# sunzeyucmu/VAE-based-Music--Deep-Generative-Models

Hardware: AMD Instinct MI355X
Metric: audio-samples/sec/GPU VQ-VAE train step, 44.1kHz 65536-frame chunks @1/2/4/8 GPU (higher is better)
Workload: dtype bf16; 1 GPU; SMALL_VQ_VAE 3-level VQ-VAE train step (BASELINE config 2); model=VQVAE levels=3 latent=64 K=2048 down_depth=[3,2,2] width=32 depth=4 dil=3, global_batch=32, seq_len=65536, parallelism=dp1, graph=True

## Files before the change

include/vqa.h:

```cpp
#ifndef VQA_H
#define VQA_H

#include <stddef.h>
#include <stdint.h>

#ifdef __cplusplus
extern "C" {
#endif

typedef void* vqa_stream_t;

enum { VQA_OK = 0, VQA_E_INVALID_ARG = -1, VQA_E_UNSUPPORTED = -2, VQA_E_HIP = -3 };
enum { VQA_F32 = 0, VQA_BF16 = 1 };

enum {
  VQA_PRE_RELU = 1,
  VQA_ADD_RESIDUAL = 2,
  VQA_POST_MASK = 4,
  VQA_X_F32 = 8,
  VQA_Y_F32 = 16
};

const char* vqa_get_last_error(void);
const char* vqa_version(void);
// ... 34 lines not shown
  float* db;
  int nparts;
  int n;
  int n_w;
  int reserved;
} vqa_partials_desc;
int vqa_conv1d_bwd_weight_partials(const void* x, const void* dy, float* dw, float* db, int B, int T_in, int T_out,
                                   int C_in, int C_out, int K, int stride, int dilation, int pad_left, int flags,
                                   int dtype, void* workspace, size_t ws_bytes, vqa_partials_desc* desc,
                                   vqa_stream_t stream);
int vqa_conv1d_transpose_bwd_weight_partials(const void* x, const void* dy, float* dw, float* db, int B, int T_in,
                                             int T_out, int C_in, int C_out, int K, int stride, int pad_left,
                                             int flags, int dtype, void* workspace, size_t ws_bytes,
                                             vqa_partials_desc* desc, vqa_stream_t stream);
int vqa_reduce_partials(const vqa_partials_desc* descs, int count, vqa_stream_t stream);

int vqa_conv1d_bwd_data_weight(const void* dy, const float* w, const void* x, const void* residual, void* dx,
                               float* dw, float* db, int B, int T_in, int T_out, int C_in, int C_out, int K,
                               int stride, int dilation, int pad_left, int flags, int dtype, void* workspace,
                               size_t ws_bytes, vqa_partials_desc* desc, vqa_stream_t stream);
size_t vqa_conv1d_bwd_data_weight_workspace(int B, int T_in, int T_out, int C_in, int C_out, int K, int stride,
                                            int dilation, int pad_left, int flags, int dtype);

enum {
  VQA_OP_FWD = 0, VQA_OP_BWD_DATA = 1, VQA_OP_BWD_WEIGHT = 2, VQA_OP_BWD_DATA_WEIGHT = 3,
  VQA_OP_T_FWD = 4, VQA_OP_T_BWD_DATA = 5, VQA_OP_T_BWD_WEIGHT = 6
};
enum {
  VQA_ROUTE_CO1 = 0, VQA_ROUTE_CONV32 = 1, VQA_ROUTE_GATHER_MFMA = 2, VQA_ROUTE_CI1 = 3, VQA_ROUTE_THIN_O = 4,
  VQA_ROUTE_THIN = 5, VQA_ROUTE_DIRECT = 6, VQA_ROUTE_WGRAD_MFMA = 7, VQA_ROUTE_WGRAD_THIN = 8,
// ... 259 lines not shown
```

vae-based-music--deep-generative-models_amd/csrc/vqa_conv.h:

```cpp
#pragma once
#include "vqa_common.h"

namespace vqa {

enum { W_DIRECT = 0, W_FLIP_T = 1, W_PAIR = 2 };

struct GatherArgs {
  const void* x;
  const float* w;
  const float* bias;
  const void* resid;
  const void* mask;
  void* y;
  int B, T_in, T_out;
  int C, O;
  int K, S, D, P;
  int wmode, Kb, Pb;
  int T_full;
  int flags;
  float* wpart = nullptr;
  int wrelu = 0;
  int wbf16 = 0;
};

// ... 58 lines not shown

enum { G_CONV32, G_MFMA, G_CI1, G_THINO, G_THIN, G_DIRECT };
struct GatherRoute {
  int family;
  int pvx;
  MfmaPlan m;
};

enum { WG_MFMA = 0, WG_THIN_X = 1, WG_THIN_G = 2, WG_DIRECT = 3 };
struct WgradPlan {
  int kind;
  int TT, CH, nchunk, nwg, E, nb;
  size_t lds, ws_bytes;
};

int gather_check(const GatherArgs& a, int dtype);
GatherRoute gather_route(const GatherArgs& a, int dtype);
int gather_nep(const GatherArgs& a, bool fw);
bool gather_thin_fits(const GatherArgs& a);
int conv32_pvx(const GatherArgs& a, int dtype, bool fw);
int run_gather(const GatherArgs& a, int dtype, hipStream_t s);
int launch_conv32_fused(const GatherArgs& a, int pvx, int dtype, hipStream_t s, int* nwg);

int wgrad_route(WgradPlan* out, int dtype, int B, int T_in, int T_out, int C, int O, int K, int S, int D, int flags);
int run_wgrad(const void* x, const void* g, float* dw, float* db, int B, int T_in, int T_out, int C, int O, int K,
              int S, int D, int P, int flags, int dtype, void* ws, size_t ws_bytes, hipStream_t s,
              vqa_partials_desc* defer);
size_t wgrad_ws(int dtype, int B, int T_in, int T_out, int C, int O, int K, int S, int D, int flags);
int reduce_partials(const float* ws, int nparts, int E, int n_w, float* dw, float* db, hipStream_t s);

}
```

vae-based-music--deep-generative-models_amd/csrc/vqa_conv.hip:

```cpp
#include "vqa_conv.h"
#include "vqa_launch.h"
#include <algorithm>

using namespace vqa;

extern "C" int vqa_same_out_len(int T_in, int stride) {
  if (stride < 1 || T_in < 0) return -1;
  return (T_in + stride - 1) / stride;
}
extern "C" int vqa_same_pad_left(int T_in, int K, int stride, int dilation) {
  if (stride < 1 || dilation < 1 || K < 1 || T_in < 0) return -1;
  const int out = (T_in + stride - 1) / stride;
  const int pad = std::max((out - 1) * stride + (K - 1) * dilation + 1 - T_in, 0);
  return pad / 2;
}

static GatherArgs conv_fwd_gather(const void* x, const float* w, const float* bias, const void* residual, void* y,
                                  int B, int T_in, int T_out, int C_in, int C_out, int K, int stride, int dilation,
                                  int pad_left, int flags) {
  return GatherArgs{x, w, bias, residual, nullptr, y, B, T_in, T_out, C_in, C_out, K, stride, dilation, pad_left,
                    W_DIRECT, K, 0, T_out, flags & (VQA_PRE_RELU | VQA_ADD_RESIDUAL | VQA_X_F32 | VQA_Y_F32)};
}

static int swap_xy_flags(int flags) {
// ... 146 lines not shown
                   conv_wgrad_flags(flags), dtype, workspace, ws_bytes, (hipStream_t)stream,
                   desc);
}

extern "C" int vqa_conv1d_transpose_bwd_weight_partials(const void* x, const void* dy, float* dw, float* db, int B,
                                                        int T_in, int T_out, int C_in, int C_out, int K, int stride,
                                                        int pad_left, int flags, int dtype, void* workspace,
                                                        size_t ws_bytes, vqa_partials_desc* desc,
                                                        vqa_stream_t stream) {
  VQA_ARG(desc, "bwd_weight_partials: NULL descriptor");
  if (const int rc = convT_check(K, stride, pad_left)) return rc;
  VQA_ARG(T_out == stride * T_in, "conv1d_transpose_bwd_weight: T_out %d != stride*T_in", T_out);
  const int f = convT_wgrad_flags(flags);
  return run_wgrad(dy, x, dw, db, B, T_out, T_in, C_out, C_in, K, stride, 1, pad_left, f, dtype, workspace, ws_bytes,
                   (hipStream_t)stream, desc);
}

static size_t fused_bwd_ws(int C_in, int C_out, int K) {
  return (size_t)cu_count() * kMaxGatherPerCU * (size_t)(K * C_in * C_out + C_out) * sizeof(float);
}

static GatherArgs fused_bwd_args(const void* dy, const float* w, const void* x, const void* residual, void* dx, int B,
                                 int T_in, int T_out, int C_in, int C_out, int K, int dilation, int pad_left,
                                 int flags) {
  const bool relu = flags & VQA_PRE_RELU;
  const int f = swap_xy_flags(flags & (VQA_ADD_RESIDUAL | VQA_X_F32 | VQA_Y_F32)) | (relu ? VQA_POST_MASK : 0);
  GatherArgs a{dy, w, nullptr, residual, x, dx, B, T_out, T_in, C_out, C_in, K, 1, dilation,
               (K - 1) * dilation - pad_left, W_FLIP_T, K, 0, T_in, f};
  a.wrelu = relu ? 1 : 0;
  return a;
// ... 205 lines not shown
```

vae-based-music--deep-generative-models_amd/csrc/vqa_conv_wgrad.hip:

```cpp
#include "vqa_conv.h"
#include "vqa_launch.h"
#include "vqa_mfma.h"

namespace vqa {

template <class T, int C, int PV>
struct RowStager {
  static constexpr int VEC = 16 / (int)sizeof(T), CPR = C / VEC;
  uint4 v[PV];
  unsigned ok;
  __device__ __forceinline__ void load(const T* Xi, int lo, int hi, int r0, int rows) {
    ok = 0u;
#pragma unroll
    for (int i = 0; i < PV; ++i) {
      const int e = threadIdx.x + i * 256;
      const int rr = e / CPR, q = e - rr * CPR, ti = r0 + rr;
      const bool val = e < rows * CPR && ti >= lo && ti < hi;
      const int tc = val ? ti : lo;
      v[i] = *((const uint4*)(Xi + (long long)tc * C) + (val ? q : 0));
      ok |= val ? (1u << i) : 0u;
    }
  }
  __device__ __forceinline__ void store(T* xl, int XS, int rows, bool relu) {
#pragma unroll
// ... 8 lines not shown
      }
    }
  }
  __device__ __forceinline__ void tail(T* xl, int XS, const T* Xi, int lo, int hi, int r0, int rows, bool relu) {
    for (int e = threadIdx.x + PV * 256; e < rows * CPR; e += 256) {
      const int rr = e / CPR, q = e - rr * CPR, ti = r0 + rr;
      uint4 t = {0u, 0u, 0u, 0u};
      if (ti >= lo && ti < hi) t = *((const uint4*)(Xi + (long long)ti * C) + q);
      if (relu) relu_bits<T>(t);
      *(uint4*)(xl + rr * XS + q * VEC) = t;
    }
  }
};

template <class T, int C, int O, int TT>
__global__ __launch_bounds__(256) void wgrad_mfma_kernel(WgradArgs a) {
  typedef Mfma<T> M;
  constexpr int XS = C + lds_pad<T>();
  constexpr int GS = O + lds_pad<T>();
  constexpr int CT = C / 16, OT = O / 16;
  constexpr int MAXTW = CT * OT;
  constexpr int KT = (int)sizeof(T) == 2 ? 32 : 4;
  extern __shared__ __attribute__((aligned(16))) char smem[];
  T* gl = (T*)smem;
  T* xl = gl + TT * GS;
  __shared__ float red[256];

  const int n = blockIdx.y, ch = blockIdx.x;
  const int tbeg = ch * a.CH, tend = min(a.T_out, tbeg + a.CH);
  const int rows_in = (TT - 1) * a.S + (a.K - 1) * a.D + 1;
  const int ntile = a.K * CT * OT;
  const int wave = __builtin_amdgcn_readfirstlane(threadIdx.x >> 6), lane = threadIdx.x & 63;

  f32x4 acc[MAXTW];
#pragma unroll
  for (int i = 0; i < MAXTW; ++i) acc[i] = f32x4{0.f, 0.f, 0.f, 0.f};
  float dbacc = 0.f;
  const bool db_x = a.flags & WG_DB_FROM_X;
  const int NB = db_x ? C : O;
  const int dbo = threadIdx.x % NB, dbr = threadIdx.x / NB, dbstep = 256 / NB;

  const bool relu = a.flags & VQA_PRE_RELU;
  const T* Gi = (const T*)a.g + (long long)n * a.T_out * O;
// ... 62 lines not shown
      for (int r = 0; r < 4; ++r) {
        const int c = ct * 16 + 4 * (lane >> 4) + r;
        out[((size_t)k * C + c) * O + o] = acc[ti][r];
      }
    }
  }
  red[threadIdx.x] = dbacc;
  __syncthreads();
  if (threadIdx.x < NB) {
    float s = 0.f;
    for (int r = 0; r < dbstep; ++r) s += red[r * NB + threadIdx.x];
    out[a.K * C * O + threadIdx.x] = s;
  }
}


template <class T> __device__ __forceinline__ float ld1_buf(__amdgpu_buffer_rsrc_t r, int off);
template <> __device__ __forceinline__ float ld1_buf<float>(__amdgpu_buffer_rsrc_t r, int off) {
  return __builtin_bit_cast(float, __builtin_amdgcn_raw_buffer_load_b32(r, off, 0, 0));
}
template <> __device__ __forceinline__ float ld1_buf<bf16>(__amdgpu_buffer_rsrc_t r, int off) {
  return __uint_as_float((unsigned)__builtin_amdgcn_raw_buffer_load_b16(r, off, 0, 0) << 16);
}
template <class T> __device__ __forceinline__ void ld8_buf(__amdgpu_buffer_rsrc_t r, int off, float* v);
template <> __device__ __forceinline__ void ld8_buf<bf16>(__amdgpu_buffer_rsrc_t r, int off, float* v) {
  const u32x4 w = __builtin_amdgcn_raw_buffer_load_b128(r, off, 0, 0);
#pragma unroll
  for (int i = 0; i < 4; ++i) {
    v[2 * i] = __uint_as_float(w[i] << 16);
    v[2 * i + 1] = __uint_as_float(w[i] & 0xFFFF0000u);
  }
}
template <> __device__ __forceinline__ void ld8_buf<float>(__amdgpu_buffer_rsrc_t r, int off, float* v) {
  const u32x4 a = __builtin_amdgcn_raw_buffer_load_b128(r, off, 0, 0);
  const u32x4 b = __builtin_amdgcn_raw_buffer_load_b128(r, off + 16, 0, 0);
#pragma unroll
  for (int i = 0; i < 4; ++i) {
    v[i] = __uint_as_float(a[i]);
    v[i + 4] = __uint_as_float(b[i]);
  }
}

template <class TX, class TG, bool WIDE_X, int NM>
__global__ __launch_bounds__(256) void wgrad_thin_kernel(WgradArgs a) {
  constexpr int KM = 4, U = 8;
  const int W = WIDE_X ? a.C : a.O;
  const int NN = WIDE_X ? a.O : a.C;
  const int VL = W / 8, RL = 256 / VL;
  const int v = threadIdx.x % VL, rl = threadIdx.x / VL;
  const int n = blockIdx.y, ch = blockIdx.x;
  const int tbeg = ch * a.CH, tend = min(a.T_out, tbeg + a.CH);
  const bool relu = a.flags & VQA_PRE_RELU;
  const unsigned xbytes = (unsigned)a.T_in * a.C * (unsigned)sizeof(TX), gbytes = (unsigned)a.T_out * a.O * (unsigned)sizeof(TG);
  const __amdgpu_buffer_rsrc_t rx = item_rsrc(a.x, (long long)n * xbytes, xbytes);
  const __amdgpu_buffer_rsrc_t rg = item_rsrc(a.g, (long long)n * gbytes, gbytes);
  float acc[KM][NM][8];
  float bacc[8];
#pragma unroll
  for (int k = 0; k < KM; ++k)
#pragma unroll
    for (int i = 0; i < NM; ++i)
#pragma unroll
      for (int j = 0; j < 8; ++j) acc[k][i][j] = 0.f;
#pragma unroll
  for (int j = 0; j < 8; ++j) bacc[j] = 0.f;
// ... 78 lines not shown
      const int o = e % a.O, c = (e / a.O) % a.C, k = e / (a.O * a.C);
      const int wide = WIDE_X ? c : o, narrow = WIDE_X ? o : c;
      vv = wide / 8;
      q = (k * NM + narrow) * 8 + (wide % 8);
    } else {
      const int o = e - KCO;
      vv = WIDE_X ? 0 : o / 8;
      q = KM * NM * 8 + (WIDE_X ? o : o % 8);
    }
    float sum = 0.f;
    for (int r = 0; r < RL; ++r) sum += red[(r * VL + vv) * PER + q];
    out[e] = sum;
  }
}

template <class TX, class TG, int TT>
__global__ __launch_bounds__(256) void wgrad_direct_kernel(WgradArgs a) {
  extern __shared__ __attribute__((aligned(16))) char smem[];
  float* gl = (float*)smem;
  float* xl = gl + TT * a.O;
  constexpr int EPT = 16;
  const int n = blockIdx.y, ch = blockIdx.x;
  const int tbeg = ch * a.CH, tend = min(a.T_out, tbeg + a.CH);
  const int rows_in = (TT - 1) * a.S + (a.K - 1) * a.D + 1;
  const int E = a.K * a.C * a.O;
  const int e0 = blockIdx.z * EPT * 256;
  const bool relu = a.flags & VQA_PRE_RELU;
  float acc[EPT];
#pragma unroll
  for (int i = 0; i < EPT; ++i) acc[i] = 0.f;
  float dbacc = 0.f;
  for (int t0 = tbeg; t0 < tend; t0 += TT) {
    const int nrows = min(TT, tend - t0);
    for (int e = threadIdx.x; e < TT * a.O; e += blockDim.x) {
      const int r = e / a.O, o = e - r * a.O;
      gl[e] = r < nrows ? ld((const TG*)a.g + ((long long)n * a.T_out + t0 + r) * a.O + o) : 0.f;
    }
    for (int e = threadIdx.x; e < rows_in * a.C; e += blockDim.x) {
      const int r = e / a.C, c = e - r * a.C;
      const int ti = t0 * a.S - a.P + r;
      float v = (ti >= 0 && ti < a.T_in) ? ld((const TX*)a.x + ((long long)n * a.T_in + ti) * a.C + c) : 0.f;
      xl[e] = relu ? fmaxf(v, 0.f) : v;
    }
    __syncthreads();
    if (blockIdx.z == 0) {
      if (a.flags & WG_DB_FROM_X) {
        if (threadIdx.x < a.C)
          for (int r = a.P; r < a.P + nrows * a.S; ++r) dbacc += xl[r * a.C + threadIdx.x];
      } else if (threadIdx.x < a.O) {
        for (int r = 0; r < nrows; ++r) dbacc += gl[r * a.O + threadIdx.x];
      }
    }
#pragma unroll
    for (int i = 0; i < EPT; ++i) {
      const int e = e0 + threadIdx.x + i * 256;
      if (e < E) {
        const int o = e % a.O, c = (e / a.O) % a.C, k = e / (a.O * a.C);
        float s = acc[i];
        for (int r = 0; r < nrows; ++r) s += xl[(r * a.S + k * a.D) * a.C + c] * gl[r * a.O + o];
        acc[i] = s;
      }
    }
    __syncthreads();
  }
  float* out = a.ws + (size_t)(n * a.nchunk + ch) * (size_t)(E + a.nb);
#pragma unroll
  for (int i = 0; i < EPT; ++i) {
    const int e = e0 + threadIdx.x + i * 256;
    if (e < E) out[e] = acc[i];
  }
  if (blockIdx.z == 0 && threadIdx.x < a.nb) out[E + threadIdx.x] = dbacc;
}

constexpr int kRedCols = 16;
__device__ __forceinline__ float reduce_col16(const float* ws, int nparts, int E, int e, float (*red)[kRedCols]) {
  const int el = threadIdx.x & (kRedCols - 1), grp = threadIdx.x / kRedCols;
  float s[8] = {0.f, 0.f, 0.f, 0.f, 0.f, 0.f, 0.f, 0.f};
  if (e < E) {
    int p = grp;
    for (; p + 7 * 16 < nparts; p += 8 * 16)
#pragma unroll
      for (int u = 0; u < 8; ++u) s[u] += ws[(size_t)(p + 16 * u) * E + e];
    for (; p < nparts; p += 16) s[0] += ws[(size_t)p * E + e];
  }
  red[grp][el] = ((s[0] + s[1]) + (s[2] + s[3])) + ((s[4] + s[5]) + (s[6] + s[7]));
  __syncthreads();
// ... 236 lines not shown
      typedef tag_t<decltype(tg)> TG;
      if (p.kind == WG_THIN_X) return launch_wgrad_thin<TX, TG, true>(a, p, s);
      if (p.kind == WG_THIN_G) return launch_wgrad_thin<TX, TG, false>(a, p, s);
      return launch_wgrad_direct<TX, TG>(a, p, s);
    });
  }
  if (rc != VQA_OK) return rc;
  const int KCO = K * C * O;
  if (defer) {
    *defer = vqa_partials_desc{(const float*)ws, dw, db, p.nwg, p.E, KCO, 0};
    return VQA_OK;
  }
  return reduce_partials((const float*)ws, p.nwg, p.E, KCO, dw, db, s);
}

size_t wgrad_ws(int dtype, int B, int T_in, int T_out, int C, int O, int K, int S, int D, int flags) {
  if (B < 1 || T_in < 1 || T_out < 1 || C < 1 || O < 1 || K < 1 || S < 1 || D < 1) return 0;
  return plan_wgrad(dtype, B, T_in, T_out, C, O, K, S, D, flags).ws_bytes;
}

}

using namespace vqa;

extern "C" int vqa_reduce_partials(const vqa_partials_desc* descs, int count, vqa_stream_t stream) {
  VQA_ARG(count >= 0 && (count == 0 || descs), "reduce_partials: bad descriptor list");
  for (int base = 0; base < count; base += kMaxDescs) {
    ReduceBatch rb{};
    rb.count = count - base < kMaxDescs ? count - base : kMaxDescs;
    int blocks = 0;
// ... 19 lines not shown
```

vae-based-music--deep-generative-models_amd/vqa_layers.py:

```python
from __future__ import annotations

import math
from typing import Dict, List, Optional, Tuple

import numpy as np
import torch

import vqa_lib as V


class ParamStore:

    ALIGN = 4

    def __init__(self):
        self.specs: List[Tuple[str, Tuple[int, ...], str]] = []
        self.offsets: Dict[str, Tuple[int, Tuple[int, ...]]] = {}
        self.size = 0
        self.count = 0
        self.flat: Optional[torch.Tensor] = None
        self.grad: Optional[torch.Tensor] = None
        self.deferred = None

    def add(self, name: str, shape: Tuple[int, ...], init: str) -> str:
# ... 158 lines not shown
    def backward_data(self, dy, T_in, cdt, mask=None, residual=None, out_dtype=None):
        B, To, _ = dy.shape
        xdt = out_dtype or cdt
        dx = torch.empty((B, T_in, self.cin), dtype=xdt, device=dy.device)
        fl = _flags_for(dx, dy.dtype, cdt) | (V.POST_MASK if mask is not None else 0) | \
            (V.ADD_RESIDUAL if residual is not None else 0)
        V.conv1d_bwd_data(dy, self.w, mask, residual, dx, B, T_in, To, self.cin, self.cout, self.K, self.s, self.d,
                          self.pad(T_in), fl, V.dtype_code(cdt))
        return dx

    def backward_weight(self, x, dy, cdt, pre_relu=False):
        B, T, _ = x.shape
        fl = _flags_for(x, dy.dtype, cdt) | (V.PRE_RELU if pre_relu else 0)
        args = (x, dy, self.store.grad_view(f"{self.name}/kernel"), self.store.grad_view(f"{self.name}/bias"), B, T,
                dy.shape[1], self.cin, self.cout, self.K, self.s, self.d, self.pad(T), fl, V.dtype_code(cdt))
        if self.store.deferred is not None:
            V.conv1d_bwd_weight_deferred(*args, self.store.deferred)
        else:
            V.conv1d_bwd_weight(*args)


    def backward_data_weight(self, dy, x, cdt, pre_relu=False, residual=None):
        B, T, _ = x.shape
        dx = torch.empty((B, T, self.cin), dtype=cdt, device=dy.device)
        fl = _flags_for(x, dy.dtype, cdt) | (V.PRE_RELU if pre_relu else 0) | \
            (V.ADD_RESIDUAL if residual is not None else 0)
        V.conv1d_bwd_data_weight(dy, self.w, x, residual, dx, self.store.grad_view(f"{self.name}/kernel"),
                                 self.store.grad_view(f"{self.name}/bias"), B, T, dy.shape[1], self.cin, self.cout,
                                 self.K, self.s, self.d, self.pad(T), fl, V.dtype_code(cdt), self.store.deferred)
        return dx


class Conv1DTranspose:

    def __init__(self, store: ParamStore, name: str, in_channels: int, filters: int, kernel_size: int,
# ... 26 lines not shown
        return y

    def backward_data(self, dy, cdt, mask=None, residual=None):
        B, To, _ = dy.shape
        T = To // self.s
        dx = torch.empty((B, T, self.cin), dtype=cdt, device=dy.device)
        fl = (V.POST_MASK if mask is not None else 0) | (V.ADD_RESIDUAL if residual is not None else 0)
        V.conv1d_transpose_bwd_data(dy, self.w, mask, residual, dx, B, T, To, self.cin, self.cout, self.K, self.s,
                                    self.pad(To), fl, V.dtype_code(cdt))
        return dx

    def backward_weight(self, x, dy, cdt):
        B, T, _ = x.shape
        args = (x, dy, self.store.grad_view(f"{self.name}/kernel"), self.store.grad_view(f"{self.name}/bias"), B, T,
                dy.shape[1], self.cin, self.cout, self.K, self.s, self.pad(dy.shape[1]), 0, V.dtype_code(cdt))
        if self.store.deferred is not None:
            V.conv1d_transpose_bwd_weight_deferred(*args, self.store.deferred)
        else:
            V.conv1d_transpose_bwd_weight(*args)
```

vae-based-music--deep-generative-models_amd/vqa_lib.py:

```python
from __future__ import annotations

import ctypes
import os
from typing import Optional

import torch

HERE = os.path.dirname(os.path.abspath(__file__))
LIB_PATH = os.environ.get("VQA_LIB_PATH") or os.path.join(HERE, "libvqa.so")

F32, BF16 = 0, 1
PRE_RELU, ADD_RESIDUAL, POST_MASK, X_F32, Y_F32 = 1, 2, 4, 8, 16

ABI_VERSION = 2

EXPORTED = [
    "vqa_get_last_error", "vqa_version", "vqa_abi_version", "vqa_same_pad_left", "vqa_same_out_len",
    "vqa_conv1d_fwd", "vqa_conv1d_bwd_data", "vqa_conv1d_bwd_weight", "vqa_conv1d_bwd_weight_workspace",
    "vqa_conv1d_transpose_fwd", "vqa_conv1d_transpose_bwd_data", "vqa_conv1d_transpose_bwd_weight",
    "vqa_conv1d_transpose_bwd_weight_workspace",
    "vqa_vq_sqnorm", "vqa_vq_argmin", "vqa_vq_quantize", "vqa_vq_quantize_workspace", "vqa_vq_backward",
    "vqa_vq_reset_rows", "vqa_vq_ema_apply", "vqa_vq_ema_apply_derived", "vqa_reset_perm_index",
    "vqa_mse_loss", "vqa_mse_loss_workspace", "vqa_adam_keras", "vqa_lr_schedule", "vqa_counter_add",
    "vqa_conv1d_bwd_weight_partials", "vqa_conv1d_transpose_bwd_weight_partials", "vqa_reduce_partials",
# ... 7 lines not shown
    "vqa_step_metrics", "vqa_synthetic_batch",
    "vqa_embedding_fwd", "vqa_embedding_bwd", "vqa_embedding_bwd_workspace", "vqa_layernorm_fwd",
    "vqa_layernorm_bwd", "vqa_layernorm_bwd_workspace",
    "vqa_seqlin_fwd", "vqa_seqlin_prep", "vqa_seqlin_fwd_prepped", "vqa_seqlin_fwd_ln_prepped", "vqa_seqlin_wgrad_workspace", "vqa_seqlin_wgrad", "vqa_prior_embed_fwd", "vqa_colsum",
    "vqa_seqlin_route", "vqa_seqlin_wgrad_plan", "vqa_head_bwd_plan",
    "vqa_axpy", "vqa_dropout", "vqa_scale_f32", "vqa_tf_mix", "vqa_attn_fwd", "vqa_attn_bwd", "vqa_head_wt",
    "vqa_head_fwd", "vqa_head_bwd_workspace", "vqa_head_bwd", "vqa_rowsum_workspace", "vqa_rowsum", "vqa_prior_decode_cache_bytes",
    "vqa_prior_decode", "vqa_prior_decode_primed", "vqa_prior_decode_filtered", "vqa_prior_decode_scored",
    "vqa_corpus_steps_per_epoch", "vqa_corpus_batch", "vqa_pcm_encode", "vqa_pcm_splice", "vqa_code_batch",
    "vqa_resample", "vqa_resample_route",
    "vqa_attn_weights_elems", "vqa_attn_weights",
    "vqa_grad_norm", "vqa_grad_norm_workspace", "vqa_adam_keras_clipped",
    "vqa_adam_keras_ema", "vqa_adam_keras_clipped_ema", "vqa_swap_f32",
    "vqa_grad_finite", "vqa_adam_keras_guarded", "vqa_counter_add_if", "vqa_step_metrics_if",
    "vqa_vq_ema_apply_guarded",
]


class VQAError(RuntimeError):
    pass


class PartialsDesc(ctypes.Structure):
    _fields_ = [("partials", ctypes.c_void_p), ("dw", ctypes.c_void_p), ("db", ctypes.c_void_p),
                ("nparts", ctypes.c_int), ("n", ctypes.c_int), ("n_w", ctypes.c_int), ("reserved", ctypes.c_int)]


_P, _I, _L, _S, _F, _U = (ctypes.c_void_p, ctypes.c_int, ctypes.c_int64, ctypes.c_size_t, ctypes.c_float,
                          ctypes.c_uint64)
_CONV = [_I] * 11
# ... 40 lines not shown
    "vqa_step_metrics_if": (_I, [_P, _P, _P, _I, _F, _P, _P]),
    "vqa_vq_ema_apply_guarded": (_I, [_P, _P, _P, _P, _P, _P, _P, _F, _F, _F, _P, _P, _P, _P, _I, _I, _P, _P]),
    "vqa_lr_schedule": (_I, [_P, _P, _I, _F, _F, _F, _F, _P]),
    "vqa_counter_add": (_I, [_P, _L, _P]),
    "vqa_step_metrics": (_I, [_P, _P, _P, _I, _F, _P]),
    "vqa_synthetic_batch": (_I, [_P, _I, _L, _U, _I, _F, _P]),
    "vqa_embedding_fwd": (_I, [_P, _P, _P, _L, _I, _I, _I, _P]),
    "vqa_embedding_bwd": (_I, [_P, _P, _P, _L, _I, _I, _I, _P, _S, _P]),
    "vqa_embedding_bwd_workspace": (_S, [_L, _I, _I]),
    "vqa_layernorm_fwd": (_I, [_P, _P, _P, _P, _L, _I, _F, _I, _P]),
    "vqa_layernorm_bwd": (_I, [_P, _P, _P, _P, _P, _P, _L, _I, _F, _I, _P, _S, _P, _P]),
    "vqa_layernorm_bwd_workspace": (_S, [_L, _I]),
    "vqa_conv1d_bwd_weight_partials": (_I, [_P, _P, _P, _P] + _CONV + [_P, _S, _P, _P]),
    "vqa_conv1d_transpose_bwd_weight_partials": (_I, [_P, _P, _P, _P] + _CONVT + [_P, _S, _P, _P]),
    "vqa_reduce_partials": (_I, [_P, _I, _P]),
    "vqa_conv1d_bwd_data_weight": (_I, [_P, _P, _P, _P, _P, _P, _P] + _CONV + [_P, _S, _P, _P]),
    "vqa_conv1d_bwd_data_weight_workspace": (_S, _CONV),
    "vqa_conv1d_route": (_I, [_I] + _CONV + [_P]),
    "vqa_spectral_loss": (_I, [_P, _P, _P, _P, _P, _I, _I, _P, _P, _P, _I, _P, _S, _P]),
    "vqa_spectral_loss_workspace": (_S, [_I, _I, _P, _P, _P, _I, _I]),
    "vqa_stft_magnitude": (_I, [_P, _P, _I, _I, _I, _I, _I, _P]),
    "vqa_vq_argmin_split": (_I, [_P, _P, _P, _P, _P, _L, _I, _I, _P]),
    "vqa_vq_split_bf16x3": (_I, [_P, _P, _I, _I, _P]),
    "vqa_resblock_supported": (_I, [_I, _I, _I]),
    "vqa_resblock_fwd": (_I, [_P] * 7 + [_I] * 5 + [_P]),
    "vqa_resblock_bwd": (_I, [_P] * 11 + [_I] * 5 + [_P, _S, _P, _P]),
    "vqa_resblock_bwd_workspace": (_S, [_I] * 5),
    "vqa_resblock_plan": (_I, [_I] * 6 + [_P]),
    "vqa_dtail_supported": (_I, [_I] * 7),
    "vqa_dtail_workspace": (_S, [_I] * 5),
# ... 146 lines not shown


def conv1d_bwd_data(dy, w, mask, residual, dx, B, T_in, T_out, C_in, C_out, K, stride, dilation, pad, flags, dtype):
    _check(lib().vqa_conv1d_bwd_data(ptr(dy), ptr(w), ptr(mask), ptr(residual), ptr(dx), B, T_in, T_out, C_in,
                                     C_out, K, stride, dilation, pad, flags, dtype, stream()), "vqa_conv1d_bwd_data")


def conv1d_bwd_weight(x, dy, dw, db, B, T_in, T_out, C_in, C_out, K, stride, dilation, pad, flags, dtype):
    n = lib().vqa_conv1d_bwd_weight_workspace(B, T_in, T_out, C_in, C_out, K, stride, dilation, pad, flags, dtype)
    ws = workspace(n, x.device)
    _check(lib().vqa_conv1d_bwd_weight(ptr(x), ptr(dy), ptr(dw), ptr(db), B, T_in, T_out, C_in, C_out, K, stride,
                                       dilation, pad, flags, dtype, ptr(ws), ws.numel(), stream()),
           "vqa_conv1d_bwd_weight")


class Deferred:

    def __init__(self):
        self.descs, self.keep = [], []

    def add(self, desc, ws):
        descs = desc if isinstance(desc, (list, tuple)) else [desc]
        self.descs.extend(descs)
        self.keep.append(ws)

    def flush(self):
        if self.descs:
            arr = (PartialsDesc * len(self.descs))(*self.descs)
            _check(lib().vqa_reduce_partials(arr, len(self.descs), stream()), "vqa_reduce_partials")
        self.descs, self.keep = [], []


def conv1d_bwd_weight_deferred(x, dy, dw, db, B, T_in, T_out, C_in, C_out, K, stride, dilation, pad, flags, dtype,
                               deferred):
    n = lib().vqa_conv1d_bwd_weight_workspace(B, T_in, T_out, C_in, C_out, K, stride, dilation, pad, flags, dtype)
    ws = workspace(n, x.device)
    d = PartialsDesc()
    _check(lib().vqa_conv1d_bwd_weight_partials(ptr(x), ptr(dy), ptr(dw), ptr(db), B, T_in, T_out, C_in, C_out, K,
                                                stride, dilation, pad, flags, dtype, ptr(ws), ws.numel(),
                                                ctypes.byref(d), stream()), "vqa_conv1d_bwd_weight_partials")
    deferred.add(d, ws)


def conv1d_bwd_data_weight(dy, w, x, residual, dx, dw, db, B, T_in, T_out, C_in, C_out, K, stride, dilation, pad,
                           flags, dtype, deferred=None):
# ... 839 lines not shown
```

Measured before the change: 335.5 million audio-samples/s.

## Group deferred conv weight-gradient kernels into batched grouped launches

Deferred weight-gradient calls are collected in Python and issued together at flush. The calls are classified by kernel variant, and each class runs as one grouped launch of up to 16 items. Each workgroup finds its item with a binary search over block offsets. This replaces many small, low-occupancy wgrad launches with fewer, larger grids, which should cut launch overhead and fill the GPU better. The cost is a kernel-argument struct holding 16 WgradArgs, extra host-side planning, and later issue of the wgrad work, which could reduce overlap with other backward kernels.

```diff
diff --git a/include/vqa.h b/include/vqa.h
--- a/include/vqa.h
+++ b/include/vqa.h
@@ -72,6 +72,27 @@
                                              int flags, int dtype, void* workspace, size_t ws_bytes,
                                              vqa_partials_desc* desc, vqa_stream_t stream);
 int vqa_reduce_partials(const vqa_partials_desc* descs, int count, vqa_stream_t stream);
+
+typedef struct {
+  const void* x;
+  const void* dy;
+  float* dw;
+  float* db;
+  int transposed;
+  int B, T_in, T_out, C_in, C_out, K, stride, dilation, pad_left, flags, dtype;
+  void* workspace;
+  size_t ws_bytes;
+} vqa_wgrad_item;
+int vqa_conv1d_wgrad_grouped(const vqa_wgrad_item* items, int count, vqa_partials_desc* descs, vqa_stream_t stream);
+int vqa_conv1d_wgrad_group_capacity(void);
+typedef struct {
+  int klass, family;
+  int first, count;
+  int blocks;
+  int64_t lds_bytes;
+} vqa_wgrad_launch;
+int vqa_conv1d_wgrad_grouped_plan(const vqa_wgrad_item* items, int count, vqa_wgrad_launch* launches,
+                                  int max_launches, int* item_index, int* item_blocks);
 
 int vqa_conv1d_bwd_data_weight(const void* dy, const float* w, const void* x, const void* residual, void* dx,
                                float* dw, float* db, int B, int T_in, int T_out, int C_in, int C_out, int K,
diff --git a/vae-based-music--deep-generative-models_amd/csrc/vqa_conv.h b/vae-based-music--deep-generative-models_amd/csrc/vqa_conv.h
--- a/vae-based-music--deep-generative-models_amd/csrc/vqa_conv.h
+++ b/vae-based-music--deep-generative-models_amd/csrc/vqa_conv.h
@@ -96,6 +96,29 @@
   size_t lds, ws_bytes;
 };
 
+struct WgradCall {
+  const void* x;
+  const void* g;
+  float* dw;
+  float* db;
+  int B, T_in, T_out, C, O, K, S, D, P, flags, dtype;
+  void* ws;
+  size_t ws_bytes;
+};
+
+constexpr int kWgradGroupCap = 16;
+
+struct WgradGroup {
+  WgradArgs a[kWgradGroupCap];
+  int start[kWgradGroupCap + 1];
+  int count;
+};
+
+struct WgradLaunch {
+  int klass, first, count, blocks;
+  size_t lds;
+};
+
 int gather_check(const GatherArgs& a, int dtype);
 GatherRoute gather_route(const GatherArgs& a, int dtype);
 int gather_nep(const GatherArgs& a, bool fw);
@@ -109,6 +132,9 @@
               int S, int D, int P, int flags, int dtype, void* ws, size_t ws_bytes, hipStream_t s,
               vqa_partials_desc* defer);
 size_t wgrad_ws(int dtype, int B, int T_in, int T_out, int C, int O, int K, int S, int D, int flags);
+int wgrad_group_plan(const WgradCall* calls, int count, WgradPlan* plans, int* order, int* blocks,
+                     WgradLaunch* launches, int max_launches, int* nlaunch);
+int run_wgrad_grouped(const WgradCall* calls, int count, vqa_partials_desc* descs, hipStream_t s);
 int reduce_partials(const float* ws, int nparts, int E, int n_w, float* dw, float* db, hipStream_t s);
 
 }
diff --git a/vae-based-music--deep-generative-models_amd/csrc/vqa_conv.hip b/vae-based-music--deep-generative-models_amd/csrc/vqa_conv.hip
--- a/vae-based-music--deep-generative-models_amd/csrc/vqa_conv.hip
+++ b/vae-based-music--deep-generative-models_amd/csrc/vqa_conv.hip
@@ -1,6 +1,7 @@
 #include "vqa_conv.h"
 #include "vqa_launch.h"
 #include <algorithm>
+#include <vector>
 
 using namespace vqa;
 
@@ -184,6 +185,58 @@
   const int f = convT_wgrad_flags(flags);
   return run_wgrad(dy, x, dw, db, B, T_out, T_in, C_out, C_in, K, stride, 1, pad_left, f, dtype, workspace, ws_bytes,
                    (hipStream_t)stream, desc);
+}
+
+static int wgrad_item_call(const vqa_wgrad_item& it, int i, WgradCall* c) {
+  if (it.transposed) {
+    if (const int rc = convT_check(it.K, it.stride, it.pad_left)) return rc;
+    VQA_ARG(it.T_out == it.stride * it.T_in, "wgrad group: item %d: T_out %d != stride*T_in", i, it.T_out);
+    *c = WgradCall{it.dy, it.x, it.dw, it.db, it.B, it.T_out, it.T_in, it.C_out, it.C_in, it.K, it.stride, 1,
+                   it.pad_left, convT_wgrad_flags(it.flags), it.dtype, it.workspace, it.ws_bytes};
+    return VQA_OK;
+  }
+  VQA_ARG(it.stride >= 1 && it.dilation >= 1 && it.K >= 1, "wgrad group: item %d: stride %d, dilation %d, K %d must be >= 1",
+          i, it.stride, it.dilation, it.K);
+  VQA_ARG(it.T_out == (it.T_in + it.stride - 1) / it.stride, "wgrad group: item %d: T_out %d != ceil(T_in/stride)", i,
+          it.T_out);
+  *c = WgradCall{it.x, it.dy, it.dw, it.db, it.B, it.T_in, it.T_out, it.C_in, it.C_out, it.K, it.stride, it.dilation,
+                 it.pad_left, conv_wgrad_flags(it.flags), it.dtype, it.workspace, it.ws_bytes};
+  return VQA_OK;
+}
+
+static int wgrad_item_calls(const vqa_wgrad_item* items, int count, std::vector<WgradCall>& calls) {
+  VQA_ARG(count >= 0 && items, "wgrad group: bad item list (count %d)", count);
+  calls.resize(count);
+  for (int i = 0; i < count; ++i)
+    if (const int rc = wgrad_item_call(items[i], i, &calls[i])) return rc;
+  return VQA_OK;
+}
+
+extern "C" int vqa_conv1d_wgrad_group_capacity(void) { return kWgradGroupCap; }
+
+extern "C" int vqa_conv1d_wgrad_grouped(const vqa_wgrad_item* items, int count, vqa_partials_desc* descs,
+                                        vqa_stream_t stream) {
+  std::vector<WgradCall> calls;
+  if (const int rc = wgrad_item_calls(items, count, calls)) return rc;
+  return run_wgrad_grouped(calls.data(), count, descs, (hipStream_t)stream);
+}
+
+extern "C" int vqa_conv1d_wgrad_grouped_plan(const vqa_wgrad_item* items, int count, vqa_wgrad_launch* launches,
+                                             int max_launches, int* item_index, int* item_blocks) {
+  std::vector<WgradCall> calls;
+  if (const int rc = wgrad_item_calls(items, count, calls)) return rc;
+  if (count == 0) return 0;
+  VQA_ARG(launches && item_index && item_blocks && max_launches >= 0, "wgrad group plan: null output");
+  std::vector<WgradPlan> plans(count);
+  std::vector<WgradLaunch> ls(count);
+  int nl = 0;
+  const int rc = wgrad_group_plan(calls.data(), count, plans.data(), item_index, item_blocks, ls.data(), count, &nl);
+  if (rc != VQA_OK) return rc;
+  VQA_ARG(nl <= max_launches, "wgrad group plan: %d launches, room for %d", nl, max_launches);
+  for (int l = 0; l < nl; ++l)
+    launches[l] = vqa_wgrad_launch{ls[l].klass, VQA_ROUTE_WGRAD_MFMA + (ls[l].klass & 3), ls[l].first, ls[l].count,
+                                   ls[l].blocks, (int64_t)ls[l].lds};
+  return nl;
 }
 
 static size_t fused_bwd_ws(int C_in, int C_out, int K) {
diff --git a/vae-based-music--deep-generative-models_amd/csrc/vqa_conv_wgrad.hip b/vae-based-music--deep-generative-models_amd/csrc/vqa_conv_wgrad.hip
--- a/vae-based-music--deep-generative-models_amd/csrc/vqa_conv_wgrad.hip
+++ b/vae-based-music--deep-generative-models_amd/csrc/vqa_conv_wgrad.hip
@@ -1,6 +1,7 @@
 #include "vqa_conv.h"
 #include "vqa_launch.h"
 #include "vqa_mfma.h"
+#include <vector>
 
 namespace vqa {
 
@@ -46,7 +47,7 @@
 };
 
 template <class T, int C, int O, int TT>
-__global__ __launch_bounds__(256) void wgrad_mfma_kernel(WgradArgs a) {
+__device__ __forceinline__ void wgrad_mfma_body(const WgradArgs& a, const int ch, const int n) {
   typedef Mfma<T> M;
   constexpr int XS = C + lds_pad<T>();
   constexpr int GS = O + lds_pad<T>();
@@ -58,7 +59,6 @@
   T* xl = gl + TT * GS;
   __shared__ float red[256];
 
-  const int n = blockIdx.y, ch = blockIdx.x;
   const int tbeg = ch * a.CH, tend = min(a.T_out, tbeg + a.CH);
   const int rows_in = (TT - 1) * a.S + (a.K - 1) * a.D + 1;
   const int ntile = a.K * CT * OT;
@@ -151,6 +151,28 @@
   }
 }
 
+template <class T, int C, int O, int TT>
+__global__ __launch_bounds__(256) void wgrad_mfma_kernel(WgradArgs a) {
+  wgrad_mfma_body<T, C, O, TT>(a, blockIdx.x, blockIdx.y);
+}
+
+__device__ __forceinline__ int group_item(const WgradGroup& g, const int b) {
+  int lo = 0, hi = g.count;
+  while (hi - lo > 1) {
+    const int mid = (lo + hi) >> 1;
+    if (b >= g.start[mid]) lo = mid; else hi = mid;
+  }
+  return lo;
+}
+
+template <class T, int C, int O, int TT>
+__global__ __launch_bounds__(256) void wgrad_mfma_grouped_kernel(WgradGroup g) {
+  const int i = group_item(g, blockIdx.x);
+  const WgradArgs& a = g.a[i];
+  const int b = (int)blockIdx.x - g.start[i];
+  wgrad_mfma_body<T, C, O, TT>(a, b % a.nchunk, b / a.nchunk);
+}
+
 
 template <class T> __device__ __forceinline__ float ld1_buf(__amdgpu_buffer_rsrc_t r, int off);
 template <> __device__ __forceinline__ float ld1_buf<float>(__amdgpu_buffer_rsrc_t r, int off) {
@@ -179,13 +201,12 @@
 }
 
 template <class TX, class TG, bool WIDE_X, int NM>
-__global__ __launch_bounds__(256) void wgrad_thin_kernel(WgradArgs a) {
+__device__ __forceinline__ void wgrad_thin_body(const WgradArgs& a, const int ch, const int n) {
   constexpr int KM = 4, U = 8;
   const int W = WIDE_X ? a.C : a.O;
   const int NN = WIDE_X ? a.O : a.C;
   const int VL = W / 8, RL = 256 / VL;
   const int v = threadIdx.x % VL, rl = threadIdx.x / VL;
-  const int n = blockIdx.y, ch = blockIdx.x;
   const int tbeg = ch * a.CH, tend = min(a.T_out, tbeg + a.CH);
   const bool relu = a.flags & VQA_PRE_RELU;
   const unsigned xbytes = (unsigned)a.T_in * a.C * (unsigned)sizeof(TX), gbytes = (unsigned)a.T_out * a.O * (unsigned)sizeof(TG);
@@ -294,17 +315,29 @@
   }
 }
 
+template <class TX, class TG, bool WIDE_X, int NM>
+__global__ __launch_bounds__(256) void wgrad_thin_kernel(WgradArgs a) {
+  wgrad_thin_body<TX, TG, WIDE_X, NM>(a, blockIdx.x, blockIdx.y);
+}
+
+template <class TX, class TG, bool WIDE_X, int NM>
+__global__ __launch_bounds__(256) void wgrad_thin_grouped_kernel(WgradGroup g) {
+  const int i = group_item(g, blockIdx.x);
+  const WgradArgs& a = g.a[i];
+  const int b = (int)blockIdx.x - g.start[i];
+  wgrad_thin_body<TX, TG, WIDE_X, NM>(a, b % a.nchunk, b / a.nchunk);
+}
+
 template <class TX, class TG, int TT>
-__global__ __launch_bounds__(256) void wgrad_direct_kernel(WgradArgs a) {
+__device__ __forceinline__ void wgrad_direct_body(const WgradArgs& a, const int ch, const int n, const int z) {
   extern __shared__ __attribute__((aligned(16))) char smem[];
   float* gl = (float*)smem;
   float* xl = gl + TT * a.O;
   constexpr int EPT = 16;
-  const int n = blockIdx.y, ch = blockIdx.x;
   const int tbeg = ch * a.CH, tend = min(a.T_out, tbeg + a.CH);
   const int rows_in = (TT - 1) * a.S + (a.K - 1) * a.D + 1;
   const int E = a.K * a.C * a.O;
-  const int e0 = blockIdx.z * EPT * 256;
+  const int e0 = z * EPT * 256;
   const bool relu = a.flags & VQA_PRE_RELU;
   float acc[EPT];
 #pragma unroll
@@ -323,7 +356,7 @@
       xl[e] = relu ? fmaxf(v, 0.f) : v;
     }
     __syncthreads();
-    if (blockIdx.z == 0) {
+    if (z == 0) {
       if (a.flags & WG_DB_FROM_X) {
         if (threadIdx.x < a.C)
           for (int r = a.P; r < a.P + nrows * a.S; ++r) dbacc += xl[r * a.C + threadIdx.x];
@@ -349,7 +382,22 @@
     const int e = e0 + threadIdx.x + i * 256;
     if (e < E) out[e] = acc[i];
   }
-  if (blockIdx.z == 0 && threadIdx.x < a.nb) out[E + threadIdx.x] = dbacc;
+  if (z == 0 && threadIdx.x < a.nb) out[E + threadIdx.x] = dbacc;
+}
+
+template <class TX, class TG, int TT>
+__global__ __launch_bounds__(256) void wgrad_direct_kernel(WgradArgs a) {
+  wgrad_direct_body<TX, TG, TT>(a, blockIdx.x, blockIdx.y, blockIdx.z);
+}
+
+template <class TX, class TG, int TT>
+__global__ __launch_bounds__(256) void wgrad_direct_grouped_kernel(WgradGroup g) {
+  const int i = group_item(g, blockIdx.x);
+  const WgradArgs& a = g.a[i];
+  const int b = (int)blockIdx.x - g.start[i];
+  const int per = a.nchunk * a.B;
+  const int r = b % per;
+  wgrad_direct_body<TX, TG, TT>(a, r % a.nchunk, r / a.nchunk, b / per);
 }
 
 constexpr int kRedCols = 16;
@@ -616,6 +664,156 @@
   return reduce_partials((const float*)ws, p.nwg, p.E, KCO, dw, db, s);
 }
 
+enum { WC_MFMA = 0, WC_THIN = 1, WC_DIRECT = 2 };
+static int wgrad_class(const WgradCall& c, const WgradPlan& p) {
+  const int xf = (c.dtype == VQA_F32 || (c.flags & VQA_X_F32)) ? 1 : 0;
+  const int gf = (c.dtype == VQA_F32 || (c.flags & VQA_Y_F32)) ? 1 : 0;
+  if (p.kind == WG_MFMA)
+    return WC_MFMA | (c.dtype == VQA_BF16 ? 4 : 0) | (c.C == 64 ? 8 : 0) | (c.O == 64 ? 16 : 0) | (p.TT == 128 ? 32 : 0);
+  if (p.kind == WG_DIRECT) return WC_DIRECT | xf << 2 | gf << 3;
+  const int wx = p.kind == WG_THIN_X ? 1 : 0;
+  const int nm2 = (wx ? c.O : c.C) == 1 ? 0 : 1;
+  return WC_THIN | xf << 2 | gf << 3 | wx << 4 | nm2 << 5;
+}
+
+static int wgrad_call_blocks(const WgradCall& c, const WgradPlan& p) {
+  const int slices = p.kind == WG_DIRECT ? (c.K * c.C * c.O + 4095) / 4096 : 1;
+  return p.nwg * slices;
+}
+
+int wgrad_group_plan(const WgradCall* calls, int count, WgradPlan* plans, int* order, int* blocks,
+                     WgradLaunch* launches, int max_launches, int* nlaunch) {
+  VQA_ARG(count >= 0 && (count == 0 || (calls && plans && order && blocks && launches)), "wgrad group: bad list");
+  *nlaunch = 0;
+  for (int i = 0; i < count; ++i) {
+    const WgradCall& c = calls[i];
+    const int rc = wgrad_route(&plans[i], c.dtype, c.B, c.T_in, c.T_out, c.C, c.O, c.K, c.S, c.D, c.flags);
+    if (rc != VQA_OK) return rc;
+    VQA_REQUIRE((long long)wgrad_call_blocks(c, plans[i]) < (1ll << 24), VQA_E_UNSUPPORTED,
+                "wgrad group: call %d has too many workgroups", i);
+  }
+  int placed = 0, nl = 0;
+  for (int i = 0; i < count; ++i) {
+    const int k = wgrad_class(calls[i], plans[i]);
+    bool seen = false;
+    for (int j = 0; j < i && !seen; ++j) seen = wgrad_class(calls[j], plans[j]) == k;
+    if (seen) continue;
+    int in_launch = kWgradGroupCap;
+    for (int j = i; j < count; ++j) {
+      if (wgrad_class(calls[j], plans[j]) != k) continue;
+      if (in_launch == kWgradGroupCap) {
+        VQA_ARG(nl < max_launches, "wgrad group: more than %d launches", max_launches);
+        launches[nl++] = WgradLaunch{k, placed, 0, 0, 0};
+        in_launch = 0;
+      }
+      WgradLaunch& L = launches[nl - 1];
+      order[placed] = j;
+      blocks[placed] = wgrad_call_blocks(calls[j], plans[j]);
+      L.blocks += blocks[placed];
+      L.lds = plans[j].lds > L.lds ? plans[j].lds : L.lds;
+      ++L.count, ++in_launch, ++placed;
+    }
+  }
+  *nlaunch = nl;
+  return VQA_OK;
+}
+
+template <class K>
+static int launch_grouped(K kernel, const char* what, const WgradGroup& g, const WgradLaunch& L, bool prepare,
+                          hipStream_t s) {
+  if (prepare) return raise_dyn_lds((const void*)kernel, L.lds, what);
+  hipLaunchKernelGGL(kernel, dim3(L.blocks), dim3(256), L.lds, s, g);
+  VQA_LAUNCHED(what);
+  return VQA_OK;
+}
+
+template <class T, int C, int O>
+static int launch_grouped_mfma_co(const WgradGroup& g, const WgradLaunch& L, bool prepare, hipStream_t s) {
+  if (L.klass & 32)
+    return launch_grouped(wgrad_mfma_grouped_kernel<T, C, O, 128>, "wgrad_mfma_grouped_kernel", g, L, prepare, s);
+  return launch_grouped(wgrad_mfma_grouped_kernel<T, C, O, 64>, "wgrad_mfma_grouped_kernel", g, L, prepare, s);
+}
+
+template <class T>
+static int launch_grouped_mfma(const WgradGroup& g, const WgradLaunch& L, bool prepare, hipStream_t s) {
+  const bool c64 = L.klass & 8, o64 = L.klass & 16;
+  if (!c64 && !o64) return launch_grouped_mfma_co<T, 32, 32>(g, L, prepare, s);
+  if (!c64 && o64) return launch_grouped_mfma_co<T, 32, 64>(g, L, prepare, s);
+  if (c64 && !o64) return launch_grouped_mfma_co<T, 64, 32>(g, L, prepare, s);
+  return launch_grouped_mfma_co<T, 64, 64>(g, L, prepare, s);
+}
+
+template <class TX, class TG, bool WX>
+static int launch_grouped_thin(const WgradGroup& g, const WgradLaunch& L, bool prepare, hipStream_t s) {
+  if (L.klass & 32)
+    return launch_grouped(wgrad_thin_grouped_kernel<TX, TG, WX, 2>, "wgrad_thin_grouped_kernel", g, L, prepare, s);
+  return launch_grouped(wgrad_thin_grouped_kernel<TX, TG, WX, 1>, "wgrad_thin_grouped_kernel", g, L, prepare, s);
+}
+
+static int launch_grouped_class(const WgradGroup& g, const WgradLaunch& L, bool prepare, hipStream_t s) {
+  const int family = L.klass & 3;
+  if (family == WC_MFMA)
+    return (L.klass & 4) ? launch_grouped_mfma<bf16>(g, L, prepare, s) : launch_grouped_mfma<float>(g, L, prepare, s);
+  return dispatch_xy(L.klass & 4, L.klass & 8, [&](auto tx, auto tg) {
+    typedef tag_t<decltype(tx)> TX;
+    typedef tag_t<decltype(tg)> TG;
+    if (family == WC_DIRECT)
+      return launch_grouped(wgrad_direct_grouped_kernel<TX, TG, 64>, "wgrad_direct_grouped_kernel", g, L, prepare, s);
+    if (L.klass & 16) return launch_grouped_thin<TX, TG, true>(g, L, prepare, s);
+    return launch_grouped_thin<TX, TG, false>(g, L, prepare, s);
+  });
+}
+
+int run_wgrad_grouped(const WgradCall* calls, int count, vqa_partials_desc* descs, hipStream_t s) {
+  VQA_ARG(count >= 0 && (count == 0 || calls), "wgrad group: bad list");
+  if (count == 0) return VQA_OK;
+  std::vector<WgradPlan> plans(count);
+  std::vector<int> order(count), blocks(count);
+  std::vector<WgradLaunch> launches(count);
+  int nl = 0;
+  int rc = wgrad_group_plan(calls, count, plans.data(), order.data(), blocks.data(), launches.data(), count, &nl);
+  if (rc != VQA_OK) return rc;
+  for (int i = 0; i < count; ++i) {
+    const WgradCall& c = calls[i];
+    VQA_ARG(c.x && c.g && c.dw, "wgrad group: call %d: null tensor pointer", i);
+    VQA_ARG(c.ws && c.ws_bytes >= plans[i].ws_bytes, "wgrad group: call %d: workspace too small: need %zu bytes, got %zu",
+            i, plans[i].ws_bytes, c.ws_bytes);
+  }
+  std::vector<WgradGroup> groups(nl);
+  for (int l = 0; l < nl; ++l) {
+    const WgradLaunch& L = launches[l];
+    WgradGroup& g = groups[l];
+    g = WgradGroup{};
+    g.count = L.count;
+    int at = 0;
+    for (int j = 0; j < L.count; ++j) {
+      const int i = order[L.first + j];
+      const WgradCall& c = calls[i];
+      const WgradPlan& p = plans[i];
+      g.a[j] = WgradArgs{c.x, c.g, (float*)c.ws, c.B, c.T_in, c.T_out, c.C, c.O, c.K, c.S, c.D, c.P, p.CH, p.nchunk,
+                         c.flags, p.nb};
+      g.start[j] = at;
+      at += blocks[L.first + j];
+    }
+    for (int j = L.count; j <= kWgradGroupCap; ++j) g.start[j] = at;
+  }
+  for (int l = 0; l < nl; ++l)
+    if ((rc = launch_grouped_class(groups[l], launches[l], true, s)) != VQA_OK) return rc;
+  for (int l = 0; l < nl; ++l)
+    if ((rc = launch_grouped_class(groups[l], launches[l], false, s)) != VQA_OK) return rc;
+  std::vector<vqa_partials_desc> local;
+  if (!descs) {
+    local.resize(count);
+    descs = local.data();
+  }
+  for (int i = 0; i < count; ++i) {
+    const WgradCall& c = calls[i];
+    descs[i] = vqa_partials_desc{(const float*)c.ws, c.dw, c.db, plans[i].nwg, plans[i].E, c.K * c.C * c.O, 0};
+  }
+  if (!local.empty()) return vqa_reduce_partials(local.data(), count, (vqa_stream_t)s);
+  return VQA_OK;
+}
+
 size_t wgrad_ws(int dtype, int B, int T_in, int T_out, int C, int O, int K, int S, int D, int flags) {
   if (B < 1 || T_in < 1 || T_out < 1 || C < 1 || O < 1 || K < 1 || S < 1 || D < 1) return 0;
   return plan_wgrad(dtype, B, T_in, T_out, C, O, K, S, D, flags).ws_bytes;
diff --git a/vae-based-music--deep-generative-models_amd/vqa_layers.py b/vae-based-music--deep-generative-models_amd/vqa_layers.py
--- a/vae-based-music--deep-generative-models_amd/vqa_layers.py
+++ b/vae-based-music--deep-generative-models_amd/vqa_layers.py
@@ -196,11 +196,12 @@
         fl = _flags_for(x, dy.dtype, cdt) | (V.PRE_RELU if pre_relu else 0)
         args = (x, dy, self.store.grad_view(f"{self.name}/kernel"), self.store.grad_view(f"{self.name}/bias"), B, T,
                 dy.shape[1], self.cin, self.cout, self.K, self.s, self.d, self.pad(T), fl, V.dtype_code(cdt))
-        if self.store.deferred is not None:
+        if self.store.deferred is not None and V.GROUP_WGRAD:
+            self.store.deferred.add_wgrad(V.wgrad_item(*args), x, dy)
+        elif self.store.deferred is not None:
             V.conv1d_bwd_weight_deferred(*args, self.store.deferred)
         else:
             V.conv1d_bwd_weight(*args)
-
 
     def backward_data_weight(self, dy, x, cdt, pre_relu=False, residual=None):
         B, T, _ = x.shape
@@ -257,7 +258,9 @@
         B, T, _ = x.shape
         args = (x, dy, self.store.grad_view(f"{self.name}/kernel"), self.store.grad_view(f"{self.name}/bias"), B, T,
                 dy.shape[1], self.cin, self.cout, self.K, self.s, self.pad(dy.shape[1]), 0, V.dtype_code(cdt))
-        if self.store.deferred is not None:
+        if self.store.deferred is not None and V.GROUP_WGRAD:
+            self.store.deferred.add_wgrad(V.wgrad_item(*args[:11], 1, *args[11:], transposed=True), x, dy)
+        elif self.store.deferred is not None:
             V.conv1d_transpose_bwd_weight_deferred(*args, self.store.deferred)
         else:
             V.conv1d_transpose_bwd_weight(*args)
diff --git a/vae-based-music--deep-generative-models_amd/vqa_lib.py b/vae-based-music--deep-generative-models_amd/vqa_lib.py
--- a/vae-based-music--deep-generative-models_amd/vqa_lib.py
+++ b/vae-based-music--deep-generative-models_amd/vqa_lib.py
@@ -45,6 +45,7 @@
     "vqa_adam_keras_ema", "vqa_adam_keras_clipped_ema", "vqa_swap_f32",
     "vqa_grad_finite", "vqa_adam_keras_guarded", "vqa_counter_add_if", "vqa_step_metrics_if",
     "vqa_vq_ema_apply_guarded",
+    "vqa_conv1d_wgrad_grouped", "vqa_conv1d_wgrad_grouped_plan", "vqa_conv1d_wgrad_group_capacity",
 ]
 
 
@@ -115,6 +116,9 @@
     "vqa_conv1d_bwd_weight_partials": (_I, [_P, _P, _P, _P] + _CONV + [_P, _S, _P, _P]),
     "vqa_conv1d_transpose_bwd_weight_partials": (_I, [_P, _P, _P, _P] + _CONVT + [_P, _S, _P, _P]),
     "vqa_reduce_partials": (_I, [_P, _I, _P]),
+    "vqa_conv1d_wgrad_grouped": (_I, [_P, _I, _P, _P]),
+    "vqa_conv1d_wgrad_grouped_plan": (_I, [_P, _I, _P, _I, _P, _P]),
+    "vqa_conv1d_wgrad_group_capacity": (_I, []),
     "vqa_conv1d_bwd_data_weight": (_I, [_P, _P, _P, _P, _P, _P, _P] + _CONV + [_P, _S, _P, _P]),
     "vqa_conv1d_bwd_data_weight_workspace": (_S, _CONV),
     "vqa_conv1d_route": (_I, [_I] + _CONV + [_P]),
@@ -291,21 +295,91 @@
            "vqa_conv1d_bwd_weight")
 
 
+class WgradItem(ctypes.Structure):
+    _fields_ = [("x", ctypes.c_void_p), ("dy", ctypes.c_void_p), ("dw", ctypes.c_void_p), ("db", ctypes.c_void_p),
+                ("transposed", ctypes.c_int), ("B", ctypes.c_int), ("T_in", ctypes.c_int), ("T_out", ctypes.c_int),
+                ("C_in", ctypes.c_int), ("C_out", ctypes.c_int), ("K", ctypes.c_int), ("stride", ctypes.c_int),
+                ("dilation", ctypes.c_int), ("pad_left", ctypes.c_int), ("flags", ctypes.c_int),
+                ("dtype", ctypes.c_int), ("workspace", ctypes.c_void_p), ("ws_bytes", ctypes.c_size_t)]
+
+
+class WgradLaunch(ctypes.Structure):
+    _fields_ = [("klass", ctypes.c_int), ("family", ctypes.c_int), ("first", ctypes.c_int), ("count", ctypes.c_int),
+                ("blocks", ctypes.c_int), ("lds_bytes", ctypes.c_int64)]
+
+
+def wgrad_item(x, dy, dw, db, B, T_in, T_out, C_in, C_out, K, stride, dilation, pad, flags, dtype, transposed=False):
+    def p(t):
+        return None if t is None else ptr(t).value
+    return WgradItem(p(x), p(dy), p(dw), p(db), int(bool(transposed)), B, T_in, T_out, C_in, C_out, K, stride,
+                     dilation, pad, flags, dtype, None, 0)
+
+
+def wgrad_item_workspace(it) -> int:
+    if it.transposed:
+        return lib().vqa_conv1d_transpose_bwd_weight_workspace(it.B, it.T_in, it.T_out, it.C_in, it.C_out, it.K,
+                                                               it.stride, it.pad_left, it.flags, it.dtype)
+    return lib().vqa_conv1d_bwd_weight_workspace(it.B, it.T_in, it.T_out, it.C_in, it.C_out, it.K, it.stride,
+                                                 it.dilation, it.pad_left, it.flags, it.dtype)
+
+
+def wgrad_group_capacity() -> int:
+    return lib().vqa_conv1d_wgrad_group_capacity()
+
+
+def conv1d_wgrad_grouped_plan(items):
+    n = len(items)
+    arr = (WgradItem * max(n, 1))(*items)
+    ls, idx, blk = (WgradLaunch * max(n, 1))(), (ctypes.c_int * max(n, 1))(), (ctypes.c_int * max(n, 1))()
+    rc = lib().vqa_conv1d_wgrad_grouped_plan(arr, n, ls, n, idx, blk)
+    if rc < 0:
+        _check(rc, "vqa_conv1d_wgrad_grouped_plan")
+    return [{"klass": L.klass, "family": ROUTE_FAMILIES[L.family], "items": list(idx[L.first:L.first + L.count]),
+             "blocks": list(blk[L.first:L.first + L.count]), "grid": L.blocks, "lds": L.lds_bytes} for L in ls[:rc]]
+
+
+def conv1d_wgrad_grouped(items, device, deferred=None):
+    n = len(items)
+    if n == 0:
+        return
+    keep = []
+    for it in items:
+        ws = workspace(wgrad_item_workspace(it), device)
+        it.workspace, it.ws_bytes = ws.data_ptr(), ws.numel()
+        keep.append(ws)
+    arr = (WgradItem * n)(*items)
+    descs = (PartialsDesc * n)() if deferred is not None else None
+    _check(lib().vqa_conv1d_wgrad_grouped(arr, n, descs, stream()), "vqa_conv1d_wgrad_grouped")
+    if deferred is not None:
+        deferred.add(list(descs), keep)
+
+
+GROUP_WGRAD = os.environ.get("VQA_GROUP_WGRAD", "1") != "0"
+
+
 class Deferred:
 
     def __init__(self):
         self.descs, self.keep = [], []
+        self.wgrads, self.wgrad_keep = [], []
 
     def add(self, desc, ws):
         descs = desc if isinstance(desc, (list, tuple)) else [desc]
         self.descs.extend(descs)
         self.keep.append(ws)
 
+    def add_wgrad(self, item, x, dy):
+        self.wgrads.append(item)
+        self.wgrad_keep.append((x, dy))
+
     def flush(self):
+        if self.wgrads:
+            conv1d_wgrad_grouped(self.wgrads, self.wgrad_keep[0][0].device, self)
         if self.descs:
             arr = (PartialsDesc * len(self.descs))(*self.descs)
             _check(lib().vqa_reduce_partials(arr, len(self.descs), stream()), "vqa_reduce_partials")
         self.descs, self.keep = [], []
+        self.wgrads, self.wgrad_keep = [], []
 
 
 def conv1d_bwd_weight_deferred(x, dy, dw, db, B, T_in, T_out, C_in, C_out, K, stride, dilation, pad, flags, dtype,
```

Result: no change. 337.8 million audio-samples/s (median of 6 runs) (+0.7%).
